# Vigilans/GomokuAI

Measured on AMD Instinct MI355X. Metric: board-evals/s, higher is better.
Workload: dtype int32; 1 GPU; batched AC-automaton position eval (K1), 65536 random-opening boards per GPU, 15x15, inputs resident in HBM; boards_per_gpu=65536, parallelism=boards sharded by rank, no collective, launch=hipGraph replay of the K steps

## Files before the change

### gomokuai_amd/csrc/eval_kernel.hip

```cpp
#include <algorithm>
#include <cstdlib>
#include <vector>

#include "capi_common.h"

namespace {

constexpr int kBoardsPerBlock = 16;
constexpr int kGroupBoards = 16;
constexpr int kThreads = 64 * kBoardsPerBlock;
constexpr int kCells = 225;
constexpr int kQueueCap = 448;
constexpr int kMaxBlocksPerCu = 1;

constexpr int kScoreWords = 4 * kCells;
constexpr int kCntWords = 3 * kCells + 1;
constexpr int kZeroWords = kScoreWords + kCntWords;
constexpr int kLineWords = 96;
constexpr int kColBase = 20, kDiagBase = 36, kAntiBase = 65;
#ifndef GMK_K1_TOTALS_COPIES
#define GMK_K1_TOTALS_COPIES 8
#endif
constexpr int kTotalsCopies = GMK_K1_TOTALS_COPIES;
constexpr int kMiscWords = 48;
constexpr int kBoardWords = kZeroWords + kLineWords + kQueueCap + kMiscWords;
static_assert(kZeroWords % 4 == 0 && kBoardWords % 4 == 0, "16-byte alignment of the per-board blocks");
constexpr int kStaticTableWords = 128 + kLineWords + 512 + 1560 + 4;

__constant__ uint32_t c_lane_jobs[64 * 2];
__constant__ uint32_t c_line_init[kLineWords];
__constant__ uint4 c_lane_consts[64];
constexpr int kScanSteps = 19;

__device__ __forceinline__ int dir_stride(int dir) { return (0x0E100F01u >> (8 * dir)) & 0xFFu; }

__device__ __forceinline__ uint64_t line_symbols(uint32_t line_word, int len) {
    return 2ull | (static_cast<uint64_t>(line_word) << 2) | (0xAull << (2 * len + 2));
}

__device__ __forceinline__ const __attribute__((address_space(3))) uint32_t* lds_word(uint32_t byte_address) {
    return reinterpret_cast<const __attribute__((address_space(3))) uint32_t*>(static_cast<uintptr_t>(byte_address));
}

__device__ __forceinline__ __attribute__((address_space(3))) uint32_t* lds_word_rw(uint32_t byte_address) {
    return reinterpret_cast<__attribute__((address_space(3))) uint32_t*>(static_cast<uintptr_t>(byte_address));
}

__device__ __forceinline__ uint32_t dfa_address(uint32_t table_word, uint32_t four) {
    uint32_t addr;
    asm("v_bfi_b32 %0, %1, %2, %3" : "=v"(addr) : "s"(0x3FF3u), "v"(table_word), "v"(four));
    return addr;
}

__device__ __forceinline__ uint32_t mul24(uint32_t a, uint32_t b) {
    uint32_t r;
    asm("v_mul_u32_u24 %0, %1, %2" : "=v"(r) : "v"(a), "s"(b));
    return r;
}

__device__ __forceinline__ void store_saddr(uint32_t byte_offset, int32_t value, unsigned long long base) {
    asm volatile("global_store_dword %0, %1, %2" : : "v"(byte_offset), "v"(value), "s"(base) : "memory");
}

template <int kImm, bool kNt>
__device__ __forceinline__ void store_saddr_imm(uint32_t byte_offset, int32_t value, unsigned long long base) {
    static_assert(kImm >= 0 && kImm < 4096, "the immediate offset of a global store has 13 bits, signed");
    if (kNt) asm volatile("global_store_dword %0, %1, %2 offset:%3 nt" : : "v"(byte_offset), "v"(value), "s"(base), "n"(kImm) : "memory");
    else asm volatile("global_store_dword %0, %1, %2 offset:%3" : : "v"(byte_offset), "v"(value), "s"(base), "n"(kImm) : "memory");
}

__device__ __forceinline__ void wave_phase_fence() {
    __builtin_amdgcn_fence(__ATOMIC_RELEASE, "wavefront");
    __builtin_amdgcn_wave_barrier();
    __builtin_amdgcn_fence(__ATOMIC_ACQUIRE, "wavefront");
}

__device__ __forceinline__ void deposit_match(uint32_t w0, uint32_t w1, int cell_at, int dir, int back_step,
                                              uint32_t* s_scores, uint32_t* s_cnt, uint32_t* s_misc, uint32_t* totals ) {
    const int type = w0 & 15, fav = (w0 >> 4) & 1;
    if (type == 8) { atomicOr(&s_misc[1], fav ? 1u : 2u); return; }
    atomicAdd(&totals[type], fav ? 0x10000u : 1u);
    const int endcell = cell_at + static_cast<int>((w0 >> 27) & 1u) * back_step;
    const uint32_t score = dir >= 2 ? (w1 >> 16) : (w1 & 0xFFFFu);
    unsigned long long* pair = reinterpret_cast<unsigned long long*>(s_scores) + fav;
    const uint32_t lo_opp = fav ? score : 0u, hi_opp = fav ? 0u : score;
    const uint32_t tslot = 5u - static_cast<uint32_t>(type);
    const bool feeds = tslot < 3u;
    uint32_t* cnt = s_cnt + (feeds ? tslot : 0u) * kCells;
    const uint32_t one = 1u << (4 * (fav * 4 + dir));
    const int n_dep = (w0 >> 8) & 7;
#pragma unroll
    for (int d = 0; d < 4; ++d) {
        if (d >= n_dep) break;
        const uint32_t f = (w0 >> (11 + 4 * d)) & 15u;
        const int c = endcell + static_cast<int>(f & 7u) * back_step;
        const bool both = (f & 8u) != 0u;
        atomicAdd(&pair[2 * c], (static_cast<unsigned long long>(both ? score : hi_opp) << 32) | (both ? score : lo_opp));
        if (both && feeds) atomicAdd(&cnt[c], one);
    }
}

__device__ __forceinline__ int counter_match(uint32_t w0, int k, int want) {
    const int type = w0 & 15, len = (w0 >> 5) & 7;
    const int back = k - static_cast<int>((w0 >> 27) & 1u) - 6;
    if (!w0 || type != want || back < 0 || back >= len) return -1;
    const int n_dep = (w0 >> 8) & 7;
    bool on_q = false;
#pragma unroll
    for (int d = 0; d < 4; ++d) {
        const uint32_t f = (w0 >> (11 + 4 * d)) & 15u;
        on_q |= d < n_dep && f == (8u | static_cast<uint32_t>(back));
    }
    return on_q ? back : -1;
}
// ... 45 lines not shown
            const int neg = __builtin_amdgcn_sbfe(static_cast<int>(occ[i / 2]), n, 1);
            store_saddr(at_black, acc[i] ^ neg, board_base);
            store_saddr(at_white, acc[i + 1] ^ neg, board_base);
            board_base += static_cast<long long>(i == 14 ? -13 : i % 4 ? 3 : 1) * (4 * 4 * plane_stride);
            asm volatile("" : "+s"(board_base));
        }
    } else {
        int32_t* out = group_out + at;
#pragma unroll
        for (int i = 0; i < 16; i += 2) {
            const int b = 4 * (i / 4) + (i % 4) / 2;
            const int neg = __builtin_amdgcn_sbfe(static_cast<int>(occ[i / 2]), n, 1);
            asm volatile("" : "+s"(n_live));
            if (b + 2 * h < n_live && plane_stride > 0) {
                out[b * 4 * plane_stride + 1 * 2 * plane_stride] = acc[i] ^ neg;
                out[b * 4 * plane_stride + 0 * 2 * plane_stride] = acc[i + 1] ^ neg;
            }
        }
    }
}

template <bool kFull>
__device__ __forceinline__ void density_planes_out(const uint16_t* __restrict__ planes, int n_boards, int first_board, int lane,
                                                   const v4i* __restrict__ s_wtab, uint32_t* __restrict__ s_occ, int32_t* __restrict__ out_density,
                                                   const uint2* __restrict__ s_lut, int plane_stride) {
    const int n = lane & 31, plane = n & 1, board = first_board + (n >> 1);
    uint32_t own[8], other[8];
    {
        const uint4* p = reinterpret_cast<const uint4*>(planes + static_cast<size_t>(kFull || board < n_boards ? board : first_board) * 32);
        const uint4 a0 = p[plane * 2], a1 = p[plane * 2 + 1], b0 = p[2 - plane * 2], b1 = p[3 - plane * 2];
        own[0] = a0.x; own[1] = a0.y; own[2] = a0.z; own[3] = a0.w; own[4] = a1.x; own[5] = a1.y; own[6] = a1.z; own[7] = a1.w;
        other[0] = b0.x; other[1] = b0.y; other[2] = b0.z; other[3] = b0.w; other[4] = b1.x; other[5] = b1.y; other[6] = b1.z; other[7] = b1.w;
    }
    if ((lane & 33) == 0) {
        const int bg = lane >> 1;
        uint32_t* slot = s_occ + 8 * ((bg >> 1) & 1) + 2 * (bg >> 2) + (bg & 1);
#pragma unroll
        for (int m = 0; m < kDensTiles; ++m) {
            const int y0 = (32 * m) / 15, y1 = (32 * m + 31) / 15;
            uint32_t occ = 0;
#pragma unroll
            for (int y = y0; y <= y1; ++y) {
                const uint32_t both = own[y / 2] | other[y / 2];
                const uint32_t r = ((y & 1) ? both >> 16 : both) & 0x7FFFu;
                const int at = 15 * y - 32 * m;
                occ |= at >= 0 ? r << at : r >> -at;
            }
            slot[16 * m] = occ;
        }
    }
    if ((lane >> 5) == 0 && (kFull || (board < n_boards && plane_stride > 0))) {
        uint32_t c224 = 0, w224 = 0;
#pragma unroll
        for (int dy = -3; dy <= 0; ++dy) {
            const int y = 14 + dy;
            const uint32_t r = (y & 1) ? own[y >> 1] >> 16 : own[y >> 1] & 0xFFFFu;
#pragma unroll
            for (int dx = -3; dx <= 0; ++dx) {
                if (block_weight(dy, dx) == 0) continue;
                const uint32_t bit = (r >> (14 + dx)) & 1u;
                c224 += bit;
                w224 += bit * static_cast<uint32_t>(block_weight(dy, dx));
            }
        }
        const uint32_t neg = 0u - (((own[7] | other[7]) >> 14) & 1u);
        int32_t* out = out_density + static_cast<size_t>(board) * 4 * plane_stride + (1 - plane) * 2 * plane_stride;
        out[224] = static_cast<int32_t>(c224 ^ neg);
        out[plane_stride + 224] = static_cast<int32_t>(w224 ^ neg);
    }
    const int n_live = __builtin_amdgcn_readfirstlane(n_boards - first_board);
    int32_t* group_out = out_density + static_cast<size_t>(first_board) * 4 * plane_stride;
    const uint4* occ_words = reinterpret_cast<const uint4*>(s_occ);
    const unsigned long long group_bits = reinterpret_cast<unsigned long long>(group_out);
    unsigned long long board_base = static_cast<unsigned long long>(static_cast<uint32_t>(__builtin_amdgcn_readfirstlane(static_cast<int>(group_bits >> 32)))) << 32
                                    | static_cast<uint32_t>(__builtin_amdgcn_readfirstlane(static_cast<int>(group_bits)));
    asm volatile("" : "+s"(board_base));
#define GMK_PASS(K, M) density_tile_pass<kFull, K, M>(own, n_live, lane, s_wtab, occ_words, group_out, board_base, s_lut, plane_stride); __builtin_amdgcn_sched_barrier(0);
    GMK_PASS(0, 0) GMK_PASS(1, 0) GMK_PASS(0, 1) GMK_PASS(1, 1) GMK_PASS(0, 2) GMK_PASS(1, 2) GMK_PASS(0, 3) GMK_PASS(1, 3)
    GMK_PASS(0, 4) GMK_PASS(1, 4) GMK_PASS(0, 5) GMK_PASS(1, 5) GMK_PASS(0, 6) GMK_PASS(1, 6)
#undef GMK_PASS
}

__global__ __launch_bounds__(kThreads)
void eval_positions_kernel(const uint16_t* __restrict__ planes, int n_boards, int n_groups,
                           int32_t* __restrict__ out_scores, int32_t* __restrict__ out_density,
                           uint32_t* __restrict__ out_totals, int32_t* __restrict__ out_status,
                           const uint32_t* __restrict__ g_trans, const uint32_t* __restrict__ g_records,
                           int trans_words, int record_words, const uint32_t* __restrict__ g_wtab,
                           int phase_mask_arg, unsigned long long* __restrict__ prof) {
#ifdef GMK_PROFILE
    const int phase_mask = phase_mask_arg;
    unsigned long long t_acc[12] = {0, 0, 0, 0, 0, 0, 0, 0, 0, 0, 0, 0}, t_prev = __builtin_amdgcn_s_memtime();
#define GMK_STAMP(k) do { if (prof) { const unsigned long long t_now_ = __builtin_amdgcn_s_memtime(); t_acc[k] += t_now_ - t_prev; t_prev = t_now_; } } while (0)
#else
    constexpr int phase_mask = 0x7F;
    (void)phase_mask_arg; (void)prof;
#ifdef GMK_K1_MARKERS
#define GMK_STAMP(k) asm volatile("; gmk_mark " #k)
#else
#define GMK_STAMP(k) do { } while (0)
#endif
#endif
    extern __shared__ __attribute__((aligned(16))) uint32_t lds[];
    const uint4* s_rec = reinterpret_cast<const uint4*>(lds + trans_words);
    uint32_t* s_jobs = lds + trans_words + record_words;

    for (int i = threadIdx.x; i < trans_words; i += kThreads) lds[i] = g_trans[i];
    for (int i = threadIdx.x; i < record_words; i += kThreads) lds[trans_words + i] = g_records[i];
    if (threadIdx.x < 128) s_jobs[threadIdx.x] = c_lane_jobs[threadIdx.x];
    uint32_t* s_pads = s_jobs + 128;
    if (threadIdx.x < kLineWords) s_pads[threadIdx.x] = ~c_line_init[threadIdx.x] & 0xAAAAAAAAu;
    uint2* s_lut = reinterpret_cast<uint2*>(s_jobs + 128 + kLineWords);
    if (threadIdx.x < 256) s_lut[threadIdx.x] = make_uint2(((threadIdx.x & 15u) * 0x204081u) & 0x01010101u, ((threadIdx.x >> 4) * 0x204081u) & 0x01010101u);
    uint32_t* s_wtab_words = s_jobs + 128 + kLineWords + 512;
    for (int i = threadIdx.x; i < kWtabWords; i += kThreads) s_wtab_words[i] = g_wtab[i];
    const v4i* s_wtab = reinterpret_cast<const v4i*>(s_wtab_words);
    uint32_t* s_handout = s_wtab_words + kWtabWords;
    if (threadIdx.x < 4) s_handout[threadIdx.x] = threadIdx.x == 0 ? 2u * kBoardsPerBlock : 0u;

    const int wave = __builtin_amdgcn_readfirstlane(threadIdx.x >> 6), lane0 = threadIdx.x & 63;
    uint32_t* s_scores = lds + trans_words + record_words + kStaticTableWords + wave * kBoardWords;
    uint32_t* s_cnt = s_scores + kScoreWords;
    uint32_t* s_lines = s_scores + kZeroWords;
    uint32_t* s_queue = s_lines + kLineWords;
    uint32_t* s_misc = s_queue + kQueueCap;
#ifndef GMK_K1_TOTALS_HOT
    uint32_t* const my_totals = s_queue + kQueueCap - 8 * kTotalsCopies + (lane0 & (kTotalsCopies - 1)) * 8;
#else
    uint32_t* const my_totals = s_misc + 4;
#endif

    GMK_STAMP(0);

    const bool planes_out = out_density != nullptr && (phase_mask & 64) && !(phase_mask & 1024);
    int lane = lane0;
    const uint32_t job_a = c_lane_jobs[lane * 2], job_b = c_lane_jobs[lane * 2 + 1];
    const uint32_t line_init_lo = c_line_init[lane], line_init_hi = c_line_init[min(64 + lane, kLineWords - 1)];
    const uint4 lane_consts = c_lane_consts[lane];
    const uint32_t cell_row4 = lane_consts.x, cell_col = lane_consts.y, norm_a = lane_consts.z, norm_b = lane_consts.w;
    uint32_t* s_rows = s_misc + 16;
    const uint16_t* row_ptr = planes + (lane & 15);
    uint32_t next_black = 0, next_white = 0, cur_black = 0, cur_white = 0;
    auto fetch_row = [&](int b) {
        const uint16_t* p = row_ptr + static_cast<size_t>(min(b, n_boards - 1)) * 32;
        next_black = p[0];
        next_white = p[16];
    };
    auto take_row = [&](int lane_m, int b) -> uint32_t { return lane_m < 16 && b < n_boards ? cur_black | (cur_white << 16) : 0u; };

    const int wg_g0 = static_cast<int>(static_cast<long long>(n_groups) * blockIdx.x / gridDim.x);
    const int wg_groups = static_cast<int>(static_cast<long long>(n_groups) * (blockIdx.x + 1) / gridDim.x) - wg_g0;
    const int wg_first = wg_g0 * kGroupBoards, wg_boards = min(wg_groups * kGroupBoards, n_boards - wg_first);
    auto hand_out = [&](int which) -> int {
        uint32_t v = 0;
        if (lane0 == 0) v = atomicAdd(&s_handout[which], 1u);
        return __builtin_amdgcn_readfirstlane(static_cast<int>(v));
    };
    int idx = wave, boards_done = 0;
    if (idx < wg_boards) fetch_row(wg_first + idx);
    asm volatile("" : "+v"(next_black), "+v"(next_white));
#pragma unroll 1
    for (;;) {
#ifdef GMK_K1_MARKERS
        GMK_STAMP(10);
#endif
        const bool live = idx < wg_boards;
        const int board = wg_first + idx;
        cur_black = next_black; cur_white = next_white;
        int idx_next = idx;
        if (live) { idx_next = boards_done == 0 ? kBoardsPerBlock + wave : hand_out(0); fetch_row(wg_first + min(idx_next, wg_boards - 1)); }
        GMK_STAMP(11);

        if (live) {
            {
                uint4* z = reinterpret_cast<uint4*>(s_cnt) + lane;
    #pragma unroll
                for (int i = 0; i < kCntWords / 4; i += 64)
                    if (i + 64 <= kCntWords / 4 || lane < kCntWords / 4 - i) z[i] = make_uint4(0u, 0u, 0u, 0u);
            }
            int lane_m = lane;
            asm volatile("" : "+v"(lane_m));
            s_lines[lane] = line_init_lo;
            if (lane_m < kLineWords - 64) s_lines[64 + lane] = line_init_hi;
            if (lane_m < kMiscWords) s_misc[lane] = 0;
#ifndef GMK_K1_TOTALS_HOT
            if (lane < 8 * kTotalsCopies) s_queue[kQueueCap - 8 * kTotalsCopies + lane] = 0;
#endif
            const uint32_t my_row = take_row(lane_m, board);
            wave_phase_fence();
            {
                uint32_t cnt = static_cast<uint32_t>(__popc(my_row & 0x7FFFu)) | (static_cast<uint32_t>(__popc(my_row >> 16)) << 16);
                cnt += static_cast<uint32_t>(__builtin_amdgcn_update_dpp(0, static_cast<int>(cnt), 0x118, 0xF, 0xF, false));
                cnt += static_cast<uint32_t>(__builtin_amdgcn_update_dpp(0, static_cast<int>(cnt), 0x114, 0xF, 0xF, false));
                cnt += static_cast<uint32_t>(__builtin_amdgcn_update_dpp(0, static_cast<int>(cnt), 0x112, 0xF, 0xF, false));
                cnt += static_cast<uint32_t>(__builtin_amdgcn_update_dpp(0, static_cast<int>(cnt), 0x111, 0xF, 0xF, false));
                if (lane_m == 15) s_misc[0] = cnt;
            }
            {
                const uint32_t r = my_row;
                const uint32_t l1 = (r & 0x3FFF3FFFu) << 1, l2 = (r & 0x1FFF1FFFu) << 2, l3 = (r & 0x0FFF0FFFu) << 3;
                const uint32_t r1 = (r & 0x7FFE7FFEu) >> 1, r2 = (r & 0x7FFC7FFCu) >> 2, r3 = (r & 0x7FF87FF8u) >> 3;
                const int far = static_cast<int>(r | l3 | r3), near = static_cast<int>(r | l1 | l2 | r1 | r2);
                uint32_t g = l1 | l2 | l3 | r1 | r2 | r3;
                g |= static_cast<uint32_t>(__builtin_amdgcn_update_dpp(0, near, 0x111, 0xF, 0xF, true)) | static_cast<uint32_t>(__builtin_amdgcn_update_dpp(0, near, 0x101, 0xF, 0xF, true));
                g |= static_cast<uint32_t>(__builtin_amdgcn_update_dpp(0, near, 0x112, 0xF, 0xF, true)) | static_cast<uint32_t>(__builtin_amdgcn_update_dpp(0, near, 0x102, 0xF, 0xF, true));
                g |= static_cast<uint32_t>(__builtin_amdgcn_update_dpp(0, far, 0x113, 0xF, 0xF, true)) | static_cast<uint32_t>(__builtin_amdgcn_update_dpp(0, far, 0x103, 0xF, 0xF, true));
                const uint32_t empty = ~(r | (r >> 16)) & 0x7FFFu;
                if (lane < 15) s_rows[3 + lane] = r;
                const int gate = static_cast<int>(g & (empty | (empty << 16)));
    #pragma unroll
                for (int pass = 0; pass < 4; ++pass) {
                    const uint32_t gw = static_cast<uint32_t>(__builtin_amdgcn_ds_bpermute(static_cast<int>((cell_row4 >> (8 * pass)) & 0xFFu), gate)) >> ((cell_col >> (8 * pass)) & 0xFFu);
                    if (pass < 3 || lane < kCells - 192)
                        reinterpret_cast<uint4*>(s_scores)[64 * pass + lane] = make_uint4(static_cast<uint32_t>(__builtin_amdgcn_sbfe(static_cast<int>(gw), 16, 1)) & 160u, 0u, 0u,
                                                                                          static_cast<uint32_t>(__builtin_amdgcn_sbfe(static_cast<int>(gw), 0, 1)) & 160u);
                }
            }
            {
                const int y = lane >> 2, part = lane & 3;
                const uint32_t row = __shfl(my_row, min(y, 14));
                uint32_t row_sym = 0;
                uint32_t y2 = 2u * static_cast<uint32_t>(y), y4 = 4u * static_cast<uint32_t>(y);
                asm volatile("" : "+v"(y2), "+v"(y4));
                for (uint32_t m = lane < 60 ? (row | (row >> 16)) & (0xFu << (4 * part)) & 0x7FFFu : 0u; m; m &= m - 1u) {
                    const int x = __ffs(m) - 1;
                    const uint32_t code = ((row >> x) & 1u) | 2u;
                    const uint32_t at_x = code << (2 * x), at_y = code << y2;
                    row_sym |= at_x;
                    char* const col = reinterpret_cast<char*>(s_lines + x);
                    atomicXor(reinterpret_cast<uint32_t*>(col) + kColBase, at_y);
                    atomicXor(reinterpret_cast<uint32_t*>(col - y4) + (kDiagBase + 14), at_x);
                    atomicXor(reinterpret_cast<uint32_t*>(col + y4) + kAntiBase, at_y);
                }
                if (row_sym) atomicXor(&s_lines[y], row_sym);
            }
            wave_phase_fence();
            GMK_STAMP(1);
        }
        if (boards_done == 0) __syncthreads();
        if (live) {
            int n_queued = 0;
            if (phase_mask & 2) {
                const int len_a = static_cast<int>(job_a & 31u) - 3, len_b = static_cast<int>(job_b & 31u) - 3;
                uint64_t syms = line_symbols(s_lines[(job_a >> 20) & 127u] >> norm_a, len_a);
                syms |= line_symbols(s_lines[(job_b >> 20) & 127u] >> norm_b, len_b) << (2 * len_a + 6);
                syms |= 0xAAAAAAAAAAAAAAAAull << (2 * (len_a + len_b) + 12);
                const uint32_t cur = static_cast<uint32_t>(syms) << 2;
                const uint32_t rest = static_cast<uint32_t>(syms >> 28);
                uint32_t tw = 0;
                const uint32_t q_base = static_cast<uint32_t>(s_queue - lds) * 4u;
                const uint32_t q_full = q_base + 4u * (kQueueCap - 64);
                uint32_t q_at = q_base;
                auto push = [&](uint32_t word, int step) {
                    const bool emits = word > 0x1FFFFu;
                    const unsigned long long emitters = __ballot(emits);
                    if (emitters) {
                        if (emits) {
                            const uint32_t ahead = __builtin_amdgcn_mbcnt_hi(static_cast<uint32_t>(emitters >> 32), __builtin_amdgcn_mbcnt_lo(static_cast<uint32_t>(emitters), 0u));
                            *lds_word_rw(q_at + 4u * ahead) = (word & ~0x1FFFFu) | (static_cast<uint32_t>(lane) | static_cast<uint32_t>(step) << 6);
                        }
                        q_at = min(q_at + 4u * static_cast<uint32_t>(__popcll(emitters)), q_full);
                    }
                };
#pragma unroll
                for (int step = 0; step < kScanSteps; ++step) {
                    const uint32_t four = step < 15 ? __builtin_amdgcn_ubfe(cur, 2 * step, 4) : __builtin_amdgcn_ubfe(rest, 2 * (step - 15), 4);
                    const uint32_t addr = dfa_address(tw, four);
                    const uint32_t before = tw;
                    tw = *lds_word(addr);
                    if (step > 0) push(before, step - 1);
                }
                push(tw, kScanSteps - 1);
                n_queued = static_cast<int>((q_at - q_base) >> 2);
                if (q_at >= q_full) s_misc[2] = 1;
            }
            wave_phase_fence();
            GMK_STAMP(2);

            if (phase_mask & 4) {
                uint32_t qe_next = s_queue[min(lane, kQueueCap - 1)];
                for (int m = lane; m < n_queued; m += 64) {
                    const uint32_t qe = qe_next;
                    qe_next = s_queue[min(m + 64, kQueueCap - 1)];
                    const int src_lane = qe & 63, src_step = (qe >> 6) & 31;
                    const uint4 rec_now = s_rec[qe >> 17];
                    const uint32_t ja_now = s_jobs[src_lane * 2], jb_now = s_jobs[src_lane * 2 + 1];
                    const int seg_a = ja_now & 31u;
                    const bool second = src_step >= seg_a;
                    const uint32_t job = second ? jb_now : ja_now;
                    const int pos = src_step - 1 - (second ? seg_a : 0);
                    const int dir = (job >> 5) & 3, stride = (job >> 7) & 31;
                    const int cell_at = static_cast<int>((job >> 12) & 255u) + pos * stride;
                    deposit_match(rec_now.x, rec_now.y, cell_at, dir, -stride, s_scores, s_cnt, s_misc, my_totals);
                    if (rec_now.z) deposit_match(rec_now.z, rec_now.w, cell_at, dir, -stride, s_scores, s_cnt, s_misc, my_totals);
                }
            }
            wave_phase_fence();
#ifndef GMK_K1_TOTALS_HOT
            if (lane < 8) {
                const uint32_t* t = s_queue + kQueueCap - 8 * kTotalsCopies + lane;
                uint32_t sum = 0;
#pragma unroll
                for (int c = 0; c < kTotalsCopies; ++c) sum += t[8 * c];
                s_misc[4 + lane] = sum;
            }
#endif
            GMK_STAMP(3);

            int n_cand = 0;
            if (phase_mask & 8) {
                uint32_t any_cnt[4];
    #pragma unroll
                for (int pass = 0; pass < 4; ++pass) {
                    const int qc = min(64 * pass + lane, kCells - 1);
                    any_cnt[pass] = s_cnt[qc] | s_cnt[kCells + qc] | s_cnt[2 * kCells + qc];
                }
    #pragma unroll
                for (int pass = 0; pass < 4; ++pass) {
                    const int q = 64 * pass + lane;
                    const uint32_t any = any_cnt[pass];
                    const uint32_t upper = (any >> 1) | (any >> 2) | (any >> 3);
                    const uint32_t clipped = ((any | upper) & 0x11111111u) + (upper & 0x11111111u);
// ... 51 lines not shown
                        if (n_comp < 2) {
                            s_misc[2] = 1;
                        } else {
                            const int ctype = min(threes, 2);
                            atomicAdd(&s_misc[12 + ctype], c ? 0x10000u : 1u);
                            const uint32_t crit = 600u * static_cast<uint32_t>(n_comp);
                            atomicAdd(reinterpret_cast<unsigned long long*>(s_scores) + 2 * q + c, (static_cast<unsigned long long>(crit) << 32) | crit);
                            queue = n_comp < 3 && !sel3;
                            const uint32_t b1 = static_cast<uint32_t>(__ffs(any_dir) - 1);
                            const uint32_t others = any_dir & (any_dir - 1u);
                            const uint32_t b2 = others ? static_cast<uint32_t>(__ffs(others) - 1) : b1;
                            const uint32_t ux = static_cast<uint32_t>(qx), uy = static_cast<uint32_t>(qy);
                            const uint32_t lines = (static_cast<uint32_t>(kColBase) << 8 | static_cast<uint32_t>(kDiagBase + 14) << 16 | static_cast<uint32_t>(kAntiBase) << 24)
                                                   + ((ux << 8) * 0x10101u) + uy * 0xFF0001u;
                            const uint32_t slots = ux * 0x0101u + uy * 0x1010u;
                            const uint32_t head = static_cast<uint32_t>(q) | (static_cast<uint32_t>(c) << 8);
                            auto entry = [&](uint32_t b) {
                                const uint32_t tslot = ((seld >> b) & 1u) ? 1u : 2u;
                                return head | (b >> 2) << 9 | tslot << 11 | __builtin_amdgcn_ubfe(lines, 2 * b, 8) << 13 | __builtin_amdgcn_ubfe(slots, b, 4) << 20;
                            };
                            ent1 = entry(b1);
                            ent2 = entry(b2);
                        }
                    }
                }
                const unsigned long long queuers = __ballot(queue);
                if (queue) {
                    const uint32_t slot = static_cast<uint32_t>(n_comp_q) + 2u * __builtin_amdgcn_mbcnt_hi(static_cast<uint32_t>(queuers >> 32),
                                                                                                          __builtin_amdgcn_mbcnt_lo(static_cast<uint32_t>(queuers), 0u));
                    s_queue[kQueueCap / 2 + slot] = ent1;
                    s_queue[kQueueCap / 2 + slot + 1] = ent2;
                }
                n_comp_q += 2 * __popcll(queuers);
                if (v0 + 64 < 2 * n_cand && n_comp_q <= kRescanFlush) continue;
            wave_phase_fence();
            GMK_STAMP(5);

            if (phase_mask & 16) {
                const int n_comp = n_comp_q;
                int lane_4 = lane;
                asm volatile("" : "+v"(lane_4));
                const int grp = lane_4 / 7, kk = lane_4 - 7 * grp, k = 6 + kk, start = k > 7 ? k - 7 : 0;
                for (int m0 = 0; m0 < n_comp; m0 += 9) {
                    const int m = m0 + grp;
                    const bool on = lane < 63 && m < n_comp;
                    const uint32_t ent = on ? s_queue[kQueueCap / 2 + m] : 0u;
                    const int q = ent & 255, c = (ent >> 8) & 1, dir = (ent >> 9) & 3, tslot = (ent >> 11) & 3;
                    const int stride = dir_stride(dir);
                    uint32_t hit_w0 = 0;
                    int hit_back = -1;
                    if (on) {
                        const uint32_t line = (ent >> 13) & 127u;
                        const uint32_t word = s_lines[line] | s_pads[line];
                        const int first = static_cast<int>((ent >> 20) & 15u) + start - 6;
                        const uint32_t cur = __builtin_amdgcn_alignbit(first >= 0 ? 0xAAAAAAAAu : word, first >= 0 ? word : 0xAAAAAAAAu,
                                                                       static_cast<uint32_t>(2 * first) & 31u) << 2;
                        uint32_t tw = 0;
    #pragma unroll
                        for (int i = 0; i < 8; ++i)
                            if (start + i <= k) tw = *lds_word(dfa_address(tw, __builtin_amdgcn_ubfe(cur, 2 * i, 4)));
                        if ((gmk::dev_trans_kinds(tw) >> tslot) & 1u) {
                            const uint4 rec = s_rec[gmk::dev_trans_record(tw)];
                            const int want = 5 - tslot;
                            hit_back = counter_match(rec.x, k, want);
                            hit_w0 = rec.x;
                            if (hit_back < 0) { hit_back = counter_match(rec.z, k, want); hit_w0 = rec.z; }
                        }
                    }
                    const unsigned long long hits = __ballot(hit_back >= 0);
                    const uint32_t mine = static_cast<uint32_t>(hits >> (7 * grp)) & 0x7Fu;
                    if (hit_back >= 0 && (mine & ((1u << kk) - 1u)) == 0u) add_counter_cells(hit_w0, hit_back, q, stride, s_scores + (c ? 2 : 1));
                }
            }
            n_comp_q = 0;
            wave_phase_fence();
            GMK_STAMP(6);
            }

        }

        asm volatile("" : "+v"(next_black), "+v"(next_white));
        GMK_STAMP(7);

        if (planes_out && (!live || (boards_done & 15) == wave)) {
            for (;;) {
                const int burst = hand_out(1);
                if (burst >= wg_groups) break;
                int lane_p = lane0, first_p = (wg_g0 + burst) * kGroupBoards;
                asm volatile("" : "+v"(lane_p), "+s"(first_p));
                const int plane_stride = (phase_mask & 512) ? 0 : (phase_mask & 256) ? 256 : kCells;
                if (first_p + kGroupBoards <= n_boards && plane_stride > 0) density_planes_out<true>(planes, n_boards, first_p, lane_p, s_wtab, s_queue, out_density, s_lut, plane_stride);
                else density_planes_out<false>(planes, n_boards, first_p, lane_p, s_wtab, s_queue, out_density, s_lut, plane_stride);
                GMK_STAMP(8);
                if (live) break;
            }
        }
        if (!live) break;
#ifdef GMK_K1_MARKERS
        GMK_STAMP(12);
#endif
        if (live && (phase_mask & 32)) {
            int lane_b = lane;
            asm volatile("" : "+v"(lane_b));
            const uint32_t lane_off = 4u * static_cast<uint32_t>(lane_b);
            if (out_scores) {
                const unsigned long long dst = reinterpret_cast<unsigned long long>(out_scores + static_cast<size_t>(board) * kScoreWords);
                const int4* src = reinterpret_cast<const int4*>(s_scores);
                const int4 v0 = src[lane_b], v1 = src[lane_b + 64], v2 = src[lane_b + 128], v3 = src[min(lane_b + 192, kCells - 1)];
#ifdef GMK_K1_PLAIN_SCORES
                constexpr bool kNt = false;
#else
                constexpr bool kNt = true;
#endif
#define GMK_STORE(words, v) store_saddr_imm<4 * (words), kNt>(lane_off, v, dst)
                const bool tail = lane_b + 192 < kCells;
                GMK_STORE(0, v0.x); GMK_STORE(64, v1.x); GMK_STORE(128, v2.x); if (tail) GMK_STORE(192, v3.x);
                GMK_STORE(kCells, v0.y); GMK_STORE(kCells + 64, v1.y); GMK_STORE(kCells + 128, v2.y); if (tail) GMK_STORE(kCells + 192, v3.y);
                GMK_STORE(2 * kCells, v0.z); GMK_STORE(2 * kCells + 64, v1.z); GMK_STORE(2 * kCells + 128, v2.z); if (tail) GMK_STORE(2 * kCells + 192, v3.z);
                GMK_STORE(3 * kCells, v0.w); GMK_STORE(3 * kCells + 64, v1.w); GMK_STORE(3 * kCells + 128, v2.w); if (tail) GMK_STORE(3 * kCells + 192, v3.w);
#undef GMK_STORE
            }
            if (out_totals) {
                const unsigned long long dst = reinterpret_cast<unsigned long long>(out_totals + static_cast<size_t>(board) * 11);
                if (lane_b < 11) store_saddr_imm<0, false>(lane_off, static_cast<int32_t>(s_misc[4 + lane_b]), dst);
            }
            if (out_status) {
                const uint32_t stones = static_cast<uint32_t>(__builtin_amdgcn_readfirstlane(static_cast<int>(s_misc[0])));
                const uint32_t wbits = static_cast<uint32_t>(__builtin_amdgcn_readfirstlane(static_cast<int>(s_misc[1])));
                const uint32_t flagged = static_cast<uint32_t>(__builtin_amdgcn_readfirstlane(static_cast<int>(s_misc[2])));
                const int stones_b = stones & 0xFFFFu, stones_w = stones >> 16;
                const int winner = (wbits & 1u) ? 1 : (wbits & 2u) ? -1 : 0;
                const bool over = winner != 0 || stones_b + stones_w == kCells;
                const int to_move = over ? 0 : (stones_b == stones_w ? 1 : -1);
                const int word = (over ? 1 : 0) | ((flagged || phase_mask != 0x7F) ? 2 : 0) | ((winner & 0xFF) << 8) | ((to_move & 0xFF) << 16);
                const unsigned long long dst = reinterpret_cast<unsigned long long>(out_status + board);
                if (lane_b == 0) store_saddr_imm<0, false>(lane_off, word, dst);
            }
        }
        wave_phase_fence();
        GMK_STAMP(9);
        idx = idx_next; ++boards_done;
    }
#ifdef GMK_PROFILE
    if (prof && lane0 == 0) {
        for (int k = 0; k < 12; ++k) atomicAdd(&prof[k], t_acc[k]);
        atomicAdd(&prof[15], 1ull);
    }
#endif
#undef GMK_STAMP
}

struct LineJob { int len, x0, y0, dir; };

int upload_lane_jobs() {
    std::vector<LineJob> lines;
    for (int i = 0; i < 15; ++i) lines.push_back({15, 0, i, 0});
    for (int i = 0; i < 15; ++i) lines.push_back({15, i, 0, 1});
    for (int d = -10; d <= 10; ++d) lines.push_back({15 - std::abs(d), d > 0 ? d : 0, d > 0 ? 0 : -d, 2});
    for (int k = 4; k <= 24; ++k) { const int x0 = std::min(k, 14); lines.push_back({std::min(k, 28 - k) + 1, x0, k - x0, 3}); }
    std::stable_sort(lines.begin(), lines.end(), [](const LineJob& a, const LineJob& b) { return a.len > b.len; });
    uint32_t jobs[128];
    for (uint32_t& j : jobs) j = 3u | (15u << 20);
    auto pack = [](const LineJob& l) {
        const int line = l.dir == 0 ? l.y0 : l.dir == 1 ? kColBase + l.x0 : l.dir == 2 ? kDiagBase + l.x0 - l.y0 + 14 : kAntiBase + l.x0 + l.y0;
        const int stride = l.dir == 0 ? 1 : l.dir == 1 ? 15 : l.dir == 2 ? 16 : 14;
        return static_cast<uint32_t>((l.len + 3) | (l.dir << 5) | (stride << 7) | ((l.y0 * 15 + l.x0) << 12) | (line << 20));
    };
    int steps = 0;
    for (int lane = 0; lane < 64; ++lane) {
        jobs[lane * 2] = pack(lines[lane]);
        int total = lines[lane].len + 3;
        const int extra = 64 + (63 - lane);
        if (extra < static_cast<int>(lines.size())) { jobs[lane * 2 + 1] = pack(lines[extra]); total += lines[extra].len + 3; }
        steps = std::max(steps, total);
    }
    uint32_t init[kLineWords] = {};
    for (int i = 0; i < 15; ++i) init[i] = init[kColBase + i] = 0x3FFFFFFFu;
    for (int d = 0; d <= 28; ++d) init[kDiagBase + d] = init[kAntiBase + d] = ((1u << (2 * (15 - std::abs(d - 14)))) - 1u) << (2 * std::max(0, d - 14));
    uint32_t consts[64][4];
    for (int lane = 0; lane < 64; ++lane) {
        uint32_t row4 = 0, col = 0;
        for (int pass = 0; pass < 4; ++pass) {
            const int c = std::min(64 * pass + lane, kCells - 1);
            row4 |= static_cast<uint32_t>(4 * (c / 15)) << (8 * pass);
            col |= static_cast<uint32_t>(c % 15) << (8 * pass);
        }
        consts[lane][0] = row4;
        consts[lane][1] = col;
        for (int k = 0; k < 2; ++k) {
            const uint32_t job = jobs[lane * 2 + k], dir = (job >> 5) & 3u, first = (job >> 12) & 255u;
            consts[lane][2 + k] = dir == 2u ? 2u * (first % 15u) : dir == 3u ? 2u * (first / 15u) : 0u;
        }
    }
    GMK_HIP_CHECK(hipMemcpyToSymbol(HIP_SYMBOL(c_lane_consts), consts, sizeof consts));
    GMK_HIP_CHECK(hipMemcpyToSymbol(HIP_SYMBOL(c_line_init), init, sizeof init));
    GMK_HIP_CHECK(hipMemcpyToSymbol(HIP_SYMBOL(c_lane_jobs), jobs, sizeof jobs));
    if (steps != kScanSteps) { gmk::set_error("lane jobs: %d scan steps, the kernel is built for %d", steps, kScanSteps); return GMK_ERR_STATE; }
    return GMK_OK;
}

int upload_density_weights(uint32_t** d_out) {
    std::vector<int8_t> t(static_cast<size_t>(kWtabWords) * 4, 0);
    for (int kind = 0; kind < 2; ++kind)
        for (int dy = -3; dy <= 3; ++dy)
            for (int xo = 0; xo < 15; ++xo)
                for (int j = 0; j < 15; ++j) {
                    if (std::abs(j - xo) > 3) continue;
                    const int w = block_weight(dy, j - xo);
                    t[((static_cast<size_t>(kind) * kWtabDy + dy + 6) * 15 + xo) * 16 + j] = static_cast<int8_t>(kind == 0 ? (w != 0) : w);
                }
    for (int cell = 0; cell < 224; ++cell)
        for (int kt = dens_kt_lo(cell / 32); kt <= dens_kt_hi(cell / 32); ++kt)
            for (int h = 0; h < 2; ++h) {
                const int dy = 2 * kt + h - cell / 15;
                if (dy < -6 || dy > 6) { gmk::set_error("density weight table: dy %d of cell %d out of range", dy, cell); return GMK_ERR_STATE; }
            }
    for (int cell = 0; cell < 224; ++cell)
        for (int dy = -3; dy <= 3; ++dy) {
            const int y = cell / 15 + dy, m = cell / 32;
            if (y < 0 || y > 14) continue;
            if (y / 2 < dens_kt_lo(m) || y / 2 > dens_kt_hi(m)) { gmk::set_error("density weight table: row %d of cell %d is not covered", y, cell); return GMK_ERR_STATE; }
        }
    GMK_HIP_CHECK(hipMalloc(d_out, t.size()));
    GMK_HIP_CHECK(hipMemcpy(*d_out, t.data(), t.size(), hipMemcpyHostToDevice));
    return GMK_OK;
}

struct Launch { int grid, n_groups; size_t lds; };

Launch plan_launch(int n, const gmk::DeviceState& st) {
    Launch l;
    l.n_groups = (n + kGroupBoards - 1) / kGroupBoards;
    l.grid = std::max(1, std::min(l.n_groups, st.cu_count * kMaxBlocksPerCu));
    l.lds = static_cast<size_t>(kBoardsPerBlock * kBoardWords + st.n_states * 4 + st.n_records * 4 + kStaticTableWords) * 4;
    return l;
}

bool g_jobs_uploaded = false;
uint32_t* g_wtab = nullptr;
}

extern "C" int gmk_eval_batch(const uint16_t* d_planes, int n, int32_t* d_scores, int32_t* d_density,
                              uint32_t* d_totals, int32_t* d_status, void* stream) {
    gmk::DeviceState& st = gmk::device_state();
    if (!st.ready) { gmk::set_error("gmk_init has not succeeded (no CPU fallback)"); return GMK_ERR_STATE; }
    if (n < 0 || (n > 0 && !d_planes)) { gmk::set_error("gmk_eval_batch: bad arguments"); return GMK_ERR_ARG; }
    if (n == 0) return GMK_OK;
    if (!g_jobs_uploaded) {
        int rc = upload_lane_jobs();
        if (rc != GMK_OK) return rc;
        rc = upload_density_weights(&g_wtab);
        if (rc != GMK_OK) return rc;
        GMK_HIP_CHECK(hipFuncSetAttribute(reinterpret_cast<const void*>(eval_positions_kernel), hipFuncAttributeMaxDynamicSharedMemorySize, 160 * 1024));
        g_jobs_uploaded = true;
    }
    const Launch l = plan_launch(n, st);
    if (l.lds > 160u * 1024u) { gmk::set_error("gmk_eval_batch: tables do not fit in LDS (%zu bytes)", l.lds); return GMK_ERR_CAPACITY; }
    static const int phase_mask = gmk::profile_env("GMK_EVAL_PHASE_MASK") ? std::atoi(gmk::profile_env("GMK_EVAL_PHASE_MASK")) : 0x7F;
    unsigned long long* d_prof = nullptr;
    static const bool stamps = gmk::profile_env("GMK_EVAL_PROFILE") != nullptr;
    if (stamps) {
        GMK_HIP_CHECK(hipMalloc(&d_prof, 16 * sizeof(unsigned long long)));
        GMK_HIP_CHECK(hipMemset(d_prof, 0, 16 * sizeof(unsigned long long)));
    }
    hipLaunchKernelGGL(eval_positions_kernel, dim3(l.grid), dim3(kThreads), l.lds, static_cast<hipStream_t>(stream),
                       d_planes, n, l.n_groups, d_scores, d_density, d_totals, d_status,
                       st.d_trans, st.d_records, st.n_states * 4, st.n_records * 4, g_wtab, phase_mask, d_prof);
    GMK_HIP_CHECK(hipGetLastError());
    if (stamps) {
        unsigned long long h[16];
        GMK_HIP_CHECK(hipDeviceSynchronize());
        GMK_HIP_CHECK(hipMemcpy(h, d_prof, sizeof h, hipMemcpyDeviceToHost));
        (void)hipFree(d_prof);
        const char* names[12] = {"staging", "phase0", "scan", "deposits", "phase3", "phase3b", "rescans", "wait-planes", "phaseD", "phase5", "-", "loop-head"};
        const double boards = static_cast<double>(n), waves = static_cast<double>(h[15] ? h[15] : 1);
        double total = 0;
        for (int k = 0; k < 12; ++k) total += static_cast<double>(h[k]);
        std::fprintf(stderr, "[GMK_EVAL_PROFILE] s_memtime cycles per board (wavefront time; %.0f wavefronts, %.0f cycles each):", waves, total / waves);
        for (int k = 0; k < 12; ++k) if (k != 10) std::fprintf(stderr, " %s %.0f", names[k], static_cast<double>(h[k]) / boards);
        std::fprintf(stderr, "\n");
    }
    return GMK_OK;
}

extern "C" int gmk_eval_launch_info(int n, int* grid, int* block, int* lds_bytes) {
    gmk::DeviceState& st = gmk::device_state();
    if (!st.ready) { gmk::set_error("gmk_init has not succeeded"); return GMK_ERR_STATE; }
    const Launch l = plan_launch(std::max(n, 1), st);
    if (grid) *grid = l.grid;
    if (block) *block = kThreads;
    if (lds_bytes) *lds_bytes = static_cast<int>(l.lds);
    return GMK_OK;
}

extern "C" int gmk_eval_batch_host(const uint16_t* h_planes, int n, int32_t* h_scores, int32_t* h_density,
                                   uint32_t* h_totals, int32_t* h_status) {
    gmk::DeviceState& st = gmk::device_state();
    if (!st.ready) { gmk::set_error("gmk_init has not succeeded (no CPU fallback)"); return GMK_ERR_STATE; }
    if (n < 0 || (n > 0 && !h_planes)) { gmk::set_error("gmk_eval_batch_host: bad arguments"); return GMK_ERR_ARG; }
    if (n == 0) return GMK_OK;
    uint16_t* d_planes = nullptr;
    int32_t *d_scores = nullptr, *d_density = nullptr, *d_status = nullptr;
    uint32_t* d_totals = nullptr;
    const size_t nb = static_cast<size_t>(n);
    int rc = GMK_OK;
    auto cleanup = [&]() { (void)hipFree(d_planes); (void)hipFree(d_scores); (void)hipFree(d_density); (void)hipFree(d_totals); (void)hipFree(d_status); };
#define GMK_TRY(expr) do { if ((expr) != hipSuccess) { gmk::set_error("%s failed", #expr); cleanup(); return GMK_ERR_HIP; } } while (0)
    GMK_TRY(hipMalloc(&d_planes, nb * 64));
    GMK_TRY(hipMalloc(&d_scores, nb * 3600));
    GMK_TRY(hipMalloc(&d_density, nb * 3600));
    GMK_TRY(hipMalloc(&d_totals, nb * 44));
    GMK_TRY(hipMalloc(&d_status, nb * 4));
    GMK_TRY(hipMemcpy(d_planes, h_planes, nb * 64, hipMemcpyHostToDevice));
    rc = gmk_eval_batch(d_planes, n, d_scores, d_density, d_totals, d_status, nullptr);
    if (rc != GMK_OK) { cleanup(); return rc; }
    GMK_TRY(hipDeviceSynchronize());
    if (h_scores) GMK_TRY(hipMemcpy(h_scores, d_scores, nb * 3600, hipMemcpyDeviceToHost));
    if (h_density) GMK_TRY(hipMemcpy(h_density, d_density, nb * 3600, hipMemcpyDeviceToHost));
    if (h_totals) GMK_TRY(hipMemcpy(h_totals, d_totals, nb * 44, hipMemcpyDeviceToHost));
    if (h_status) GMK_TRY(hipMemcpy(h_status, d_status, nb * 4, hipMemcpyDeviceToHost));
#undef GMK_TRY
    cleanup();
    return GMK_OK;
}
```

Baseline: 560.6 million board-evals/s.

## Stage all K1 tables from one prebuilt image and schedule density bursts statically

All LDS tables (transitions, records, lane jobs, pads, LUT, density weights, handout counter) are now packed on the host into one device image. Each block copies that image with 16-byte vector loads, and the first two vectors per thread are issued before the first board fetch. Per-lane constants come from the same global buffer instead of __constant__ memory, and the per-block group split is precomputed on the host. The dynamically handed-out density-plane bursts are replaced by a fixed rule: the wave holding board idx, where idx is a multiple of 12, writes burst idx/12. This removes a second atomic counter but may balance the work across waves less evenly. A profiling-only timeline dump is also added.

```diff
diff --git a/gomokuai_amd/csrc/eval_kernel.hip b/gomokuai_amd/csrc/eval_kernel.hip
--- a/gomokuai_amd/csrc/eval_kernel.hip
+++ b/gomokuai_amd/csrc/eval_kernel.hip
@@ -12,6 +12,9 @@
 constexpr int kCells = 225;
 constexpr int kQueueCap = 448;
 constexpr int kMaxBlocksPerCu = 1;
+constexpr int kBurstEvery = 12;
+static_assert(kBurstEvery >= 1 && kBurstEvery <= kGroupBoards, "every burst of a run needs a board of the run to go with");
+[[maybe_unused]] constexpr int kTimelineSlots = 8;
 
 constexpr int kScoreWords = 4 * kCells;
 constexpr int kCntWords = 3 * kCells + 1;
@@ -27,9 +30,7 @@
 static_assert(kZeroWords % 4 == 0 && kBoardWords % 4 == 0, "16-byte alignment of the per-board blocks");
 constexpr int kStaticTableWords = 128 + kLineWords + 512 + 1560 + 4;
 
-__constant__ uint32_t c_lane_jobs[64 * 2];
-__constant__ uint32_t c_line_init[kLineWords];
-__constant__ uint4 c_lane_consts[64];
+constexpr int kLaneRecordVecs = 2;
 constexpr int kScanSteps = 19;
 
 __device__ __forceinline__ int dir_stride(int dir) { return (0x0E100F01u >> (8 * dir)) & 0xFFu; }
@@ -241,19 +242,24 @@
 }
 
 __global__ __launch_bounds__(kThreads)
-void eval_positions_kernel(const uint16_t* __restrict__ planes, int n_boards, int n_groups,
+void eval_positions_kernel(const uint16_t* __restrict__ planes, int n_boards, int groups_each, int groups_extra,
                            int32_t* __restrict__ out_scores, int32_t* __restrict__ out_density,
                            uint32_t* __restrict__ out_totals, int32_t* __restrict__ out_status,
-                           const uint32_t* __restrict__ g_trans, const uint32_t* __restrict__ g_records,
-                           int trans_words, int record_words, const uint32_t* __restrict__ g_wtab,
-                           int phase_mask_arg, unsigned long long* __restrict__ prof) {
+                           const uint4* __restrict__ g_stage, int stage_vecs, int trans_words, int record_words,
+                           int phase_mask_arg, unsigned long long* __restrict__ prof, unsigned long long* __restrict__ timeline) {
 #ifdef GMK_PROFILE
+    unsigned long long* const tl_row = timeline ? timeline + (static_cast<size_t>(blockIdx.x) * kBoardsPerBlock + (threadIdx.x >> 6)) * kTimelineSlots : nullptr;
+#define GMK_TL(slot, value) do { if (tl_row && (threadIdx.x & 63) == 0) tl_row[slot] = (value); } while (0)
+    GMK_TL(0, __builtin_amdgcn_s_memtime());
+    unsigned long long tl_last_board = 0, tl_burst_clocks = 0;
+    int tl_bursts = 0;
     const int phase_mask = phase_mask_arg;
     unsigned long long t_acc[12] = {0, 0, 0, 0, 0, 0, 0, 0, 0, 0, 0, 0}, t_prev = __builtin_amdgcn_s_memtime();
 #define GMK_STAMP(k) do { if (prof) { const unsigned long long t_now_ = __builtin_amdgcn_s_memtime(); t_acc[k] += t_now_ - t_prev; t_prev = t_now_; } } while (0)
 #else
     constexpr int phase_mask = 0x7F;
-    (void)phase_mask_arg; (void)prof;
+    (void)phase_mask_arg; (void)prof; (void)timeline;
+#define GMK_TL(slot, value) do { } while (0)
 #ifdef GMK_K1_MARKERS
 #define GMK_STAMP(k) asm volatile("; gmk_mark " #k)
 #else
@@ -264,18 +270,15 @@
     const uint4* s_rec = reinterpret_cast<const uint4*>(lds + trans_words);
     uint32_t* s_jobs = lds + trans_words + record_words;
 
-    for (int i = threadIdx.x; i < trans_words; i += kThreads) lds[i] = g_trans[i];
-    for (int i = threadIdx.x; i < record_words; i += kThreads) lds[trans_words + i] = g_records[i];
-    if (threadIdx.x < 128) s_jobs[threadIdx.x] = c_lane_jobs[threadIdx.x];
+    const int tid = threadIdx.x;
+    const uint4 stage_a = g_stage[min(tid, stage_vecs - 1)], stage_b = g_stage[min(tid + kThreads, stage_vecs - 1)];
+    const uint4* lane_record = g_stage + stage_vecs + kLaneRecordVecs * (tid & 63);
+    const uint4 lane_lines = lane_record[0], lane_consts = lane_record[1];
     uint32_t* s_pads = s_jobs + 128;
-    if (threadIdx.x < kLineWords) s_pads[threadIdx.x] = ~c_line_init[threadIdx.x] & 0xAAAAAAAAu;
     uint2* s_lut = reinterpret_cast<uint2*>(s_jobs + 128 + kLineWords);
-    if (threadIdx.x < 256) s_lut[threadIdx.x] = make_uint2(((threadIdx.x & 15u) * 0x204081u) & 0x01010101u, ((threadIdx.x >> 4) * 0x204081u) & 0x01010101u);
     uint32_t* s_wtab_words = s_jobs + 128 + kLineWords + 512;
-    for (int i = threadIdx.x; i < kWtabWords; i += kThreads) s_wtab_words[i] = g_wtab[i];
     const v4i* s_wtab = reinterpret_cast<const v4i*>(s_wtab_words);
     uint32_t* s_handout = s_wtab_words + kWtabWords;
-    if (threadIdx.x < 4) s_handout[threadIdx.x] = threadIdx.x == 0 ? 2u * kBoardsPerBlock : 0u;
 
     const int wave = __builtin_amdgcn_readfirstlane(threadIdx.x >> 6), lane0 = threadIdx.x & 63;
     uint32_t* s_scores = lds + trans_words + record_words + kStaticTableWords + wave * kBoardWords;
@@ -293,9 +296,8 @@
 
     const bool planes_out = out_density != nullptr && (phase_mask & 64) && !(phase_mask & 1024);
     int lane = lane0;
-    const uint32_t job_a = c_lane_jobs[lane * 2], job_b = c_lane_jobs[lane * 2 + 1];
-    const uint32_t line_init_lo = c_line_init[lane], line_init_hi = c_line_init[min(64 + lane, kLineWords - 1)];
-    const uint4 lane_consts = c_lane_consts[lane];
+    const uint32_t job_a = lane_lines.x, job_b = lane_lines.y;
+    const uint32_t line_init_lo = lane_lines.z, line_init_hi = lane_lines.w;
     const uint32_t cell_row4 = lane_consts.x, cell_col = lane_consts.y, norm_a = lane_consts.z, norm_b = lane_consts.w;
     uint32_t* s_rows = s_misc + 16;
     const uint16_t* row_ptr = planes + (lane & 15);
@@ -307,17 +309,25 @@
     };
     auto take_row = [&](int lane_m, int b) -> uint32_t { return lane_m < 16 && b < n_boards ? cur_black | (cur_white << 16) : 0u; };
 
-    const int wg_g0 = static_cast<int>(static_cast<long long>(n_groups) * blockIdx.x / gridDim.x);
-    const int wg_groups = static_cast<int>(static_cast<long long>(n_groups) * (blockIdx.x + 1) / gridDim.x) - wg_g0;
+    const int wg_block = static_cast<int>(blockIdx.x);
+    const int wg_g0 = groups_each * wg_block + min(wg_block, groups_extra);
+    const int wg_groups = groups_each + (wg_block < groups_extra ? 1 : 0);
     const int wg_first = wg_g0 * kGroupBoards, wg_boards = min(wg_groups * kGroupBoards, n_boards - wg_first);
-    auto hand_out = [&](int which) -> int {
+    auto hand_out = [&]() -> int {
         uint32_t v = 0;
-        if (lane0 == 0) v = atomicAdd(&s_handout[which], 1u);
+        if (lane0 == 0) v = atomicAdd(s_handout, 1u);
         return __builtin_amdgcn_readfirstlane(static_cast<int>(v));
     };
     int idx = wave, boards_done = 0;
     if (idx < wg_boards) fetch_row(wg_first + idx);
+    {
+        uint4* s_stage = reinterpret_cast<uint4*>(lds);
+        if (tid < stage_vecs) s_stage[tid] = stage_a;
+        if (tid + kThreads < stage_vecs) s_stage[tid + kThreads] = stage_b;
+        for (int i = tid + 2 * kThreads; i < stage_vecs; i += kThreads) s_stage[i] = g_stage[i];
+    }
     asm volatile("" : "+v"(next_black), "+v"(next_white));
+    GMK_TL(1, __builtin_amdgcn_s_memtime());
 #pragma unroll 1
     for (;;) {
 #ifdef GMK_K1_MARKERS
@@ -327,7 +337,7 @@
         const int board = wg_first + idx;
         cur_black = next_black; cur_white = next_white;
         int idx_next = idx;
-        if (live) { idx_next = boards_done == 0 ? kBoardsPerBlock + wave : hand_out(0); fetch_row(wg_first + min(idx_next, wg_boards - 1)); }
+        if (live) { idx_next = boards_done == 0 ? kBoardsPerBlock + wave : hand_out(); fetch_row(wg_first + min(idx_next, wg_boards - 1)); }
         GMK_STAMP(11);
 
         if (live) {
@@ -396,7 +406,14 @@
             wave_phase_fence();
             GMK_STAMP(1);
         }
+#ifdef GMK_PROFILE
+        if (boards_done == 0) GMK_TL(2, __builtin_amdgcn_s_memtime());
+#endif
         if (boards_done == 0) __syncthreads();
+#ifdef GMK_PROFILE
+        if (boards_done == 0) GMK_TL(3, __builtin_amdgcn_s_memtime());
+        if (live) { tl_bursts = 0; tl_burst_clocks = 0; }
+#endif
         if (live) {
             int n_queued = 0;
             if (phase_mask & 2) {
@@ -614,20 +631,22 @@
         asm volatile("" : "+v"(next_black), "+v"(next_white));
         GMK_STAMP(7);
 
-        if (planes_out && (!live || (boards_done & 15) == wave)) {
-            for (;;) {
-                const int burst = hand_out(1);
-                if (burst >= wg_groups) break;
-                int lane_p = lane0, first_p = (wg_g0 + burst) * kGroupBoards;
-                asm volatile("" : "+v"(lane_p), "+s"(first_p));
-                const int plane_stride = (phase_mask & 512) ? 0 : (phase_mask & 256) ? 256 : kCells;
-                if (first_p + kGroupBoards <= n_boards && plane_stride > 0) density_planes_out<true>(planes, n_boards, first_p, lane_p, s_wtab, s_queue, out_density, s_lut, plane_stride);
-                else density_planes_out<false>(planes, n_boards, first_p, lane_p, s_wtab, s_queue, out_density, s_lut, plane_stride);
-                GMK_STAMP(8);
-                if (live) break;
-            }
-        }
         if (!live) break;
+        const int burst = idx / kBurstEvery;
+        if (planes_out && burst * kBurstEvery == idx && burst < wg_groups) {
+#ifdef GMK_PROFILE
+            const unsigned long long tl_burst_from = __builtin_amdgcn_s_memtime();
+#endif
+            int lane_p = lane0, first_p = (wg_g0 + burst) * kGroupBoards;
+            asm volatile("" : "+v"(lane_p), "+s"(first_p));
+            const int plane_stride = (phase_mask & 512) ? 0 : (phase_mask & 256) ? 256 : kCells;
+            if (first_p + kGroupBoards <= n_boards && plane_stride > 0) density_planes_out<true>(planes, n_boards, first_p, lane_p, s_wtab, s_queue, out_density, s_lut, plane_stride);
+            else density_planes_out<false>(planes, n_boards, first_p, lane_p, s_wtab, s_queue, out_density, s_lut, plane_stride);
+            GMK_STAMP(8);
+#ifdef GMK_PROFILE
+            ++tl_bursts; tl_burst_clocks += __builtin_amdgcn_s_memtime() - tl_burst_from;
+#endif
+        }
 #ifdef GMK_K1_MARKERS
         GMK_STAMP(12);
 #endif
@@ -671,20 +690,28 @@
         }
         wave_phase_fence();
         GMK_STAMP(9);
+#ifdef GMK_PROFILE
+        tl_last_board = __builtin_amdgcn_s_memtime();
+#endif
         idx = idx_next; ++boards_done;
     }
 #ifdef GMK_PROFILE
+    GMK_TL(4, tl_last_board);
+    GMK_TL(6, static_cast<unsigned long long>(tl_bursts) | static_cast<unsigned long long>(boards_done) << 16);
+    GMK_TL(7, tl_burst_clocks);
+    GMK_TL(5, __builtin_amdgcn_s_memtime());
     if (prof && lane0 == 0) {
         for (int k = 0; k < 12; ++k) atomicAdd(&prof[k], t_acc[k]);
         atomicAdd(&prof[15], 1ull);
     }
 #endif
 #undef GMK_STAMP
+#undef GMK_TL
 }
 
 struct LineJob { int len, x0, y0, dir; };
 
-int upload_lane_jobs() {
+int lane_tables(uint32_t* jobs_out, uint32_t* pads_out, uint32_t* records_out) {
     std::vector<LineJob> lines;
     for (int i = 0; i < 15; ++i) lines.push_back({15, 0, i, 0});
     for (int i = 0; i < 15; ++i) lines.push_back({15, i, 0, 1});
@@ -724,15 +751,19 @@
             consts[lane][2 + k] = dir == 2u ? 2u * (first % 15u) : dir == 3u ? 2u * (first / 15u) : 0u;
         }
     }
-    GMK_HIP_CHECK(hipMemcpyToSymbol(HIP_SYMBOL(c_lane_consts), consts, sizeof consts));
-    GMK_HIP_CHECK(hipMemcpyToSymbol(HIP_SYMBOL(c_line_init), init, sizeof init));
-    GMK_HIP_CHECK(hipMemcpyToSymbol(HIP_SYMBOL(c_lane_jobs), jobs, sizeof jobs));
+    for (int i = 0; i < 128; ++i) jobs_out[i] = jobs[i];
+    for (int i = 0; i < kLineWords; ++i) pads_out[i] = ~init[i] & 0xAAAAAAAAu;
+    for (int lane = 0; lane < 64; ++lane) {
+        uint32_t* r = records_out + 8 * lane;
+        r[0] = jobs[lane * 2]; r[1] = jobs[lane * 2 + 1];
+        r[2] = init[lane]; r[3] = init[std::min(64 + lane, kLineWords - 1)];
+        for (int k = 0; k < 4; ++k) r[4 + k] = consts[lane][k];
+    }
     if (steps != kScanSteps) { gmk::set_error("lane jobs: %d scan steps, the kernel is built for %d", steps, kScanSteps); return GMK_ERR_STATE; }
     return GMK_OK;
 }
 
-int upload_density_weights(uint32_t** d_out) {
-    std::vector<int8_t> t(static_cast<size_t>(kWtabWords) * 4, 0);
+int density_weights(int8_t* t ) {
     for (int kind = 0; kind < 2; ++kind)
         for (int dy = -3; dy <= 3; ++dy)
             for (int xo = 0; xo < 15; ++xo)
@@ -753,23 +784,46 @@
             if (y < 0 || y > 14) continue;
             if (y / 2 < dens_kt_lo(m) || y / 2 > dens_kt_hi(m)) { gmk::set_error("density weight table: row %d of cell %d is not covered", y, cell); return GMK_ERR_STATE; }
         }
-    GMK_HIP_CHECK(hipMalloc(d_out, t.size()));
-    GMK_HIP_CHECK(hipMemcpy(*d_out, t.data(), t.size(), hipMemcpyHostToDevice));
     return GMK_OK;
 }
 
-struct Launch { int grid, n_groups; size_t lds; };
+int build_stage_image(const gmk::DeviceState& st, uint4** d_out, int* stage_vecs) {
+    const size_t trans_words = static_cast<size_t>(st.n_states) * 4, record_words = static_cast<size_t>(st.n_records) * 4;
+    std::vector<uint32_t> rest(kStaticTableWords + 64 * 4 * kLaneRecordVecs, 0u);
+    uint32_t* jobs = rest.data(), *pads = jobs + 128, *lut = pads + kLineWords, *wtab = lut + 512, *handout = wtab + kWtabWords, *records = handout + 4;
+    int rc = lane_tables(jobs, pads, records);
+    if (rc != GMK_OK) return rc;
+    for (uint32_t b = 0; b < 256; ++b) { lut[2 * b] = ((b & 15u) * 0x204081u) & 0x01010101u; lut[2 * b + 1] = ((b >> 4) * 0x204081u) & 0x01010101u; }
+    rc = density_weights(reinterpret_cast<int8_t*>(wtab));
+    if (rc != GMK_OK) return rc;
+    handout[0] = 2u * kBoardsPerBlock;
+    const size_t staged_words = trans_words + record_words + kStaticTableWords;
+    if (staged_words % 4 != 0) { gmk::set_error("K1 tables: %zu staged words are not whole 16-byte pieces", staged_words); return GMK_ERR_STATE; }
+    uint32_t* d = nullptr;
+    GMK_HIP_CHECK(hipMalloc(&d, (trans_words + record_words + rest.size()) * sizeof(uint32_t)));
+    GMK_HIP_CHECK(hipMemcpy(d, st.d_trans, trans_words * sizeof(uint32_t), hipMemcpyDeviceToDevice));
+    GMK_HIP_CHECK(hipMemcpy(d + trans_words, st.d_records, record_words * sizeof(uint32_t), hipMemcpyDeviceToDevice));
+    GMK_HIP_CHECK(hipMemcpy(d + trans_words + record_words, rest.data(), rest.size() * sizeof(uint32_t), hipMemcpyHostToDevice));
+    *d_out = reinterpret_cast<uint4*>(d);
+    *stage_vecs = static_cast<int>(staged_words / 4);
+    return GMK_OK;
+}
+
+struct Launch { int grid, n_groups, groups_each, groups_extra; size_t lds; };
 
 Launch plan_launch(int n, const gmk::DeviceState& st) {
     Launch l;
     l.n_groups = (n + kGroupBoards - 1) / kGroupBoards;
     l.grid = std::max(1, std::min(l.n_groups, st.cu_count * kMaxBlocksPerCu));
+    l.groups_each = l.n_groups / l.grid;
+    l.groups_extra = l.n_groups % l.grid;
     l.lds = static_cast<size_t>(kBoardsPerBlock * kBoardWords + st.n_states * 4 + st.n_records * 4 + kStaticTableWords) * 4;
     return l;
 }
 
 bool g_jobs_uploaded = false;
-uint32_t* g_wtab = nullptr;
+uint4* g_stage = nullptr;
+int g_stage_vecs = 0;
 }
 
 extern "C" int gmk_eval_batch(const uint16_t* d_planes, int n, int32_t* d_scores, int32_t* d_density,
@@ -779,9 +833,7 @@
     if (n < 0 || (n > 0 && !d_planes)) { gmk::set_error("gmk_eval_batch: bad arguments"); return GMK_ERR_ARG; }
     if (n == 0) return GMK_OK;
     if (!g_jobs_uploaded) {
-        int rc = upload_lane_jobs();
-        if (rc != GMK_OK) return rc;
-        rc = upload_density_weights(&g_wtab);
+        const int rc = build_stage_image(st, &g_stage, &g_stage_vecs);
         if (rc != GMK_OK) return rc;
         GMK_HIP_CHECK(hipFuncSetAttribute(reinterpret_cast<const void*>(eval_positions_kernel), hipFuncAttributeMaxDynamicSharedMemorySize, 160 * 1024));
         g_jobs_uploaded = true;
@@ -795,10 +847,33 @@
         GMK_HIP_CHECK(hipMalloc(&d_prof, 16 * sizeof(unsigned long long)));
         GMK_HIP_CHECK(hipMemset(d_prof, 0, 16 * sizeof(unsigned long long)));
     }
+    static const char* const timeline_path = gmk::profile_env("GMK_EVAL_TIMELINE");
+    unsigned long long* d_timeline = nullptr;
+    const size_t timeline_words = static_cast<size_t>(l.grid) * kBoardsPerBlock * kTimelineSlots;
+    hipEvent_t tl_from = nullptr, tl_to = nullptr;
+    if (timeline_path) {
+        GMK_HIP_CHECK(hipMalloc(&d_timeline, timeline_words * sizeof(unsigned long long)));
+        GMK_HIP_CHECK(hipMemset(d_timeline, 0, timeline_words * sizeof(unsigned long long)));
+        GMK_HIP_CHECK(hipEventCreate(&tl_from));
+        GMK_HIP_CHECK(hipEventCreate(&tl_to));
+        GMK_HIP_CHECK(hipDeviceSynchronize());
+        GMK_HIP_CHECK(hipEventRecord(tl_from, static_cast<hipStream_t>(stream)));
+    }
     hipLaunchKernelGGL(eval_positions_kernel, dim3(l.grid), dim3(kThreads), l.lds, static_cast<hipStream_t>(stream),
-                       d_planes, n, l.n_groups, d_scores, d_density, d_totals, d_status,
-                       st.d_trans, st.d_records, st.n_states * 4, st.n_records * 4, g_wtab, phase_mask, d_prof);
+                       d_planes, n, l.groups_each, l.groups_extra, d_scores, d_density, d_totals, d_status,
+                       g_stage, g_stage_vecs, st.n_states * 4, st.n_records * 4, phase_mask, d_prof, d_timeline);
     GMK_HIP_CHECK(hipGetLastError());
+    if (timeline_path) {
+        GMK_HIP_CHECK(hipEventRecord(tl_to, static_cast<hipStream_t>(stream)));
+        GMK_HIP_CHECK(hipEventSynchronize(tl_to));
+        float wall_ms = 0.f;
+        GMK_HIP_CHECK(hipEventElapsedTime(&wall_ms, tl_from, tl_to));
+        std::vector<unsigned long long> h(4 + timeline_words);
+        h[0] = static_cast<unsigned long long>(l.grid); h[1] = kBoardsPerBlock; h[2] = kTimelineSlots; h[3] = static_cast<unsigned long long>(wall_ms * 1e6);
+        GMK_HIP_CHECK(hipMemcpy(h.data() + 4, d_timeline, timeline_words * sizeof(unsigned long long), hipMemcpyDeviceToHost));
+        (void)hipFree(d_timeline); (void)hipEventDestroy(tl_from); (void)hipEventDestroy(tl_to);
+        if (std::FILE* f = std::fopen(timeline_path, "wb")) { std::fwrite(h.data(), sizeof(unsigned long long), h.size(), f); std::fclose(f); }
+    }
     if (stamps) {
         unsigned long long h[16];
         GMK_HIP_CHECK(hipDeviceSynchronize());
```

Result: faster. 579.9 million board-evals/s (median of 6 runs) (+3.4%).
